# PRBonn/OverlapNet

Measured on NVIDIA H100. Metric: scan-pairs/sec (overlap+yaw) at 64x900, higher is better.
Workload: dtype f16

## Files before the change

overlapnet_b200/csrc/network_tc.cu:

```cuda
#include "common.cuh"
#include "hopper.cuh"

#include <cuda_fp16.h>
#include <stddef.h>
#include <stdlib.h>

namespace ovn {

using namespace hopper;

constexpr int WF = 360;
constexpr int CF = 128;
constexpr int S15 = 15;
constexpr int NB = 24;
constexpr int PAIR_ROWS = NB * NB;
constexpr int K4_PITCH = CF;

struct TcState {
  Buffer<__half> w1p;
  Buffer<__half> w2p;
  Buffer<__half> w3p;
  Buffer<float> b2eff;
  Buffer<__half> wres[kMaxLegLayers];
  Buffer<__half> actp[2];
// ... 23 lines not shown
};

void TcStateDelete::operator()(TcState* t) const { delete t; }

__host__ __device__ __forceinline__ int k4_pos(int r, int c) {
  const int k = c & 31;
  return (((c >> 5) ^ (r & 1)) << 5) + ((k & 7) >> 1) * 8 + (k >> 3) * 2 + (k & 1);
}

__device__ __forceinline__ bool h2_nonfinite(__half2 v) {
  const uint32_t b = *reinterpret_cast<const uint32_t*>(&v);
  return (b & 0x7c00u) == 0x7c00u || (b & 0x7c000000u) == 0x7c000000u;
}

__global__ void __launch_bounds__(256)
k_gather_rows_f16(const float* __restrict__ bank, const int32_t* __restrict__ idx, int n, const float* __restrict__ mu,
                  int row_shift, __half* __restrict__ out, int* __restrict__ err, int32_t* __restrict__ row_bad) {
  const int64_t per = (int64_t)WF * CF / 4;
  const int64_t i = (int64_t)blockIdx.x * blockDim.x + threadIdx.x;
  if (i >= (int64_t)n * per) return;
  const int p = (int)(i / per);
  const int64_t e = i % per;
  const int64_t row = idx ? idx[p] : p;
  const int r = (int)(e / (CF / 4)), c4 = (int)(e % (CF / 4));
  int64_t rs = r + row_shift;
  if (rs >= WF) rs -= WF;
  const float4 v = __ldg(reinterpret_cast<const float4*>(bank + (row * WF + rs) * CF) + c4);
  const float4 m = __ldg(reinterpret_cast<const float4*>(mu) + c4);
  __half2 a = __floats2half2_rn(v.x - m.x, v.y - m.y), b = __floats2half2_rn(v.z - m.z, v.w - m.w);
  if (h2_nonfinite(a) || h2_nonfinite(b)) {
    if (row_bad) row_bad[p] = 1;
    else atomicCAS(err, 0, kErrNonFiniteOperand);
  }
  __half* o = out + ((int64_t)p * WF + r) * K4_PITCH;
  *reinterpret_cast<uint32_t*>(o + k4_pos(r, 4 * c4)) = *reinterpret_cast<uint32_t*>(&a);
  *reinterpret_cast<uint32_t*>(o + k4_pos(r, 4 * c4 + 2)) = *reinterpret_cast<uint32_t*>(&b);
}

__global__ void __launch_bounds__(1024)
k_channel_mean(const float* __restrict__ bank, const int32_t* __restrict__ idx, int n, float* __restrict__ mu) {
  __shared__ float part[8][CF];
  const int c = threadIdx.x & (CF - 1), g = threadIdx.x >> 7;
  float acc = 0.f;
  for (int v = 0; v < n; ++v) {
    const float* vol = bank + (int64_t)(idx ? idx[v] : v) * WF * CF;
    for (int r = g; r < WF; r += 8) acc += __ldg(vol + (int64_t)r * CF + c);
  }
  part[g][c] = acc;
  __syncthreads();
  if (g == 0) {
    float t = 0.f;
    for (int k = 0; k < 8; ++k) t += part[k][c];
    mu[c] = __half2float(__float2half_rn(t / (float)((int64_t)n * WF)));
  }
}

constexpr int K4_STEPS = 60;

__host__ __device__ __forceinline__ size_t o1_row_offset(int64_t m, int di) {
  return ((size_t)((m >> 7) * S15 + di) * 128 + (size_t)(m & 127)) * 64;
}
__host__ __device__ __forceinline__ size_t o1_chunk_offset(int64_t m, int di, int c8) {
  return o1_row_offset(m, di) + (size_t)((c8 ^ (int)(m & 7)) * 8);
}

struct LegArgs {
  const __half* A; int64_t a_pitch;
  int runs_per_img, in_img_planes, in_run_planes;
  int kh, kw, c8in;
  const __half* Bp;
  const float* bias; int n_valid;
  int64_t M;
  __half* out_planes; int64_t out_pitch; int out_run_planes;
  float* out_f32;
  int n_split; float* part;
  int* err;
};

__device__ __forceinline__ bool leg_act_unstorable(float v) { return !(v < 65520.f) || v == -INFINITY; }

constexpr int C6_LROWS = 64, C6_RROWS = 128;
constexpr int C6_LT = 6, C6_RT = 3;
constexpr int C6_L_BYTES = 2 * 16 * C6_LROWS * 16;
constexpr int C6_R_BYTES = 2 * 16 * C6_RROWS * 16;
constexpr int C6_VOL_L_BYTES = C6_LT * C6_L_BYTES;
constexpr int C6_VOL_R_BYTES = C6_RT * C6_R_BYTES;

template <int TR, int NT>
__global__ void __launch_bounds__(256)
k_pack_corr(const float* __restrict__ bank, const int32_t* __restrict__ idx, int n, __half* __restrict__ out,
            int* __restrict__ err, int32_t* __restrict__ row_bad) {
  const int64_t i = (int64_t)blockIdx.x * blockDim.x + threadIdx.x;
  const int64_t per = 16 * NT * TR;
  if (i >= (int64_t)n * per) return;
  const int p = (int)(i / per);
  int r = (int)(i % per);
  const int vrow = r % (NT * TR); r /= NT * TR;
  const int pl = r;
  const int tile = vrow / TR, row = vrow % TR;
  float v[8];
  if (vrow < WF) {
    const int64_t src = (idx ? idx[p] : p);
    const float4 a = __ldg(reinterpret_cast<const float4*>(bank + (src * WF + vrow) * CF + pl * 8));
    const float4 b = __ldg(reinterpret_cast<const float4*>(bank + (src * WF + vrow) * CF + pl * 8 + 4));
    v[0] = a.x; v[1] = a.y; v[2] = a.z; v[3] = a.w; v[4] = b.x; v[5] = b.y; v[6] = b.z; v[7] = b.w;
  } else {
#pragma unroll
    for (int e = 0; e < 8; ++e) v[e] = 0.f;
  }
  __half hi[8], lo[8];
#pragma unroll
  for (int e = 0; e < 8; ++e) {
    hi[e] = __float2half_rn(v[e]);
    lo[e] = __float2half_rn(v[e] - __half2float(hi[e]));
  }
  bool bad = false;
#pragma unroll
  for (int e = 0; e < 8; e += 2) bad |= h2_nonfinite(__halves2half2(hi[e], hi[e + 1]));
  if (bad) {
    if (row_bad) row_bad[p] = 1;
    else atomicCAS(err, 0, kErrNonFiniteOperand);
  }
  __half* base = out + ((size_t)p * NT + tile) * (2 * 16 * TR * 8);
  *reinterpret_cast<uint4*>(base + ((size_t)pl * TR + row) * 8) = *reinterpret_cast<const uint4*>(hi);
  *reinterpret_cast<uint4*>(base + ((size_t)(16 + pl) * TR + row) * 8) = *reinterpret_cast<const uint4*>(lo);
}

constexpr int MMA_THREADS = 128;
constexpr int MMA_ROWS = 64;

__device__ __forceinline__ void mma16816(float (&d)[4], uint32_t a0, uint32_t a1, uint32_t a2, uint32_t a3,
                                         uint32_t b0, uint32_t b1) {
  asm volatile("mma.sync.aligned.m16n8k16.row.col.f32.f16.f16.f32 {%0,%1,%2,%3}, {%4,%5,%6,%7}, {%8,%9}, {%0,%1,%2,%3};"
               : "+f"(d[0]), "+f"(d[1]), "+f"(d[2]), "+f"(d[3])
               : "r"(a0), "r"(a1), "r"(a2), "r"(a3), "r"(b0), "r"(b1));
}

__device__ __forceinline__ uint32_t ld_h2(const __half* p) { return __ldg(reinterpret_cast<const unsigned int*>(p)); }

__device__ __forceinline__ uint32_t absdiff_h2(uint32_t a, uint32_t b) {
  const __half2 d = __hsub2(*reinterpret_cast<const __half2*>(&a), *reinterpret_cast<const __half2*>(&b));
  return *reinterpret_cast<const uint32_t*>(&d) & 0x7fff7fffu;
}

__device__ __forceinline__ uint32_t pack_h2(float a, float b) {
  const __half2 h = __floats2half2_rn(a, b);
  return *reinterpret_cast<const uint32_t*>(&h);
}

constexpr int K4_WG = 3;
constexpr int K4_THREADS = (K4_WG + 1) * 128;
constexpr uint32_t K4_REG_PRODUCER = 32, K4_REG_CONSUMER = 160;
constexpr int K4_GROUP = 5;
constexpr int K4_NGROUPS = K4_STEPS / K4_GROUP;
static_assert(S15 % K4_GROUP == 0, "a W1 group within one 32-channel chunk");
constexpr int K4_RING = 4;
constexpr int K4_BSLICE = 4096;
constexpr uint32_t K4_VOL_BYTES = WF * K4_PITCH * 2;
constexpr uint32_t K4_RWIN_BYTES = S15 * K4_PITCH * 2;
constexpr int K4_O1S_PITCH = NB * 64 + 8;

struct K4Smem {
  __half L[WF * K4_PITCH];
  __half Rw[2][S15 * K4_PITCH];
  __half B[K4_RING][K4_GROUP * K4_BSLICE / 2];
  __half O1s[S15 * K4_O1S_PITCH];
  MbarRing<K4_RING> w1;
  MbarRing<1> left;
  MbarRing<2> right;
  MbarRing<1> o1s;
};
static_assert(sizeof(K4Smem) <= 232448, "k_delta_conv1_wgmma shared memory");
static_assert(offsetof(K4Smem, B) % 16 == 0 && offsetof(K4Smem, Rw) % 16 == 0 && offsetof(K4Smem, O1s) % 16 == 0 &&
              K4_O1S_PITCH * 2 % 16 == 0, "bulk-copy alignment");

struct Share { int64_t begin, end; };
__device__ __forceinline__ Share work_share(int64_t n, uint32_t part, uint32_t parts) {
  return {n * part / parts, n * (part + 1) / parts};
}

__global__ void __launch_bounds__(K4_THREADS, 1)
k_delta_conv1_wgmma(const __half* __restrict__ L16, const int32_t* __restrict__ l_idx, const __half* __restrict__ R16,
                    int r_per_pair, const __half* __restrict__ W1p, const float* __restrict__ mu_o1,
                    __half* __restrict__ o1, int n_pairs, int* __restrict__ err) {
  extern __shared__ __align__(128) uint8_t smem_raw[];
  K4Smem& S = *reinterpret_cast<K4Smem*>(smem_raw);
  const int tid = threadIdx.x, warp = tid >> 5, lane = tid & 31;
  const Share share = work_share((int64_t)n_pairs * NB, blockIdx.x, gridDim.x);
  const int u_begin = (int)share.begin, u_end = (int)share.end;
  if (tid == 0) {
    S.w1.init(K4_WG * 4);
    S.left.init(K4_WG * 4);
    S.right.init(K4_WG * 4);
    S.o1s.init(1, K4_WG * 4);
    mbar_fence_init();
  }
  __syncthreads();

  if (warp >= K4_WG * 4) {
    setmaxnreg_dec<K4_REG_PRODUCER>();
    if (warp == K4_WG * 4 && lane == 0) {
      uint32_t pi = 0, gi = 0, ui = 0;
      for (int u = u_begin; u < u_end; ++u, ++ui) {
        const int p = u / NB, jb = u - p * NB;
        if (u == u_begin || jb == 0) {
          PIPE_WAIT(S.left.acquire(pi, K4_VOL_BYTES), kErrDeltaLeftProducer);
          bulk_g2s(S.L, L16 + (size_t)(l_idx ? l_idx[p] : p) * WF * K4_PITCH, K4_VOL_BYTES, S.left.bar(pi));
          ++pi;
        }
        PIPE_WAIT(S.right.acquire(ui, K4_RWIN_BYTES), kErrDeltaRightProducer);
        bulk_g2s(S.Rw[S.right.slot(ui)], R16 + (r_per_pair ? (size_t)p * WF * K4_PITCH : 0) + (size_t)jb * S15 * K4_PITCH,
                 K4_RWIN_BYTES, S.right.bar(ui));
        for (int grp = 0; grp < K4_NGROUPS; ++grp, ++gi) {
          PIPE_WAIT(S.w1.acquire(gi, K4_GROUP * K4_BSLICE), kErrDeltaW1Producer);
          bulk_g2s(S.B[S.w1.slot(gi)], W1p + (size_t)grp * K4_GROUP * (K4_BSLICE / 2), K4_GROUP * K4_BSLICE, S.w1.bar(gi));
        }
      }
    } else if (warp == K4_WG * 4 + 1 && lane == 0) {
      uint32_t ui = 0;
      for (int u = u_begin; u < u_end; ++u, ++ui) {
        const int p = u / NB, jb = u - p * NB;
        const int64_t m0 = (int64_t)p * PAIR_ROWS + jb * NB;
        const int n0 = min(NB, 128 - (int)(m0 & 127));
        if (!S.o1s.wait(ui)) { atomicExch(err, kErrDeltaO1Producer); break; }
#pragma unroll 1
        for (int di = 0; di < S15; ++di) {
          const __half* src = S.O1s + di * K4_O1S_PITCH;
          bulk_s2g(o1 + o1_row_offset(m0, di), src, n0 * 128);
          if (n0 < NB) bulk_s2g(o1 + o1_row_offset(m0 + n0, di), src + n0 * 64, (NB - n0) * 128);
        }
        bulk_commit();
        bulk_wait_read<0>();
        S.o1s.release_thread(ui);
      }
      bulk_wait<0>();
    }
  } else {
    setmaxnreg_inc<K4_REG_CONSUMER>();
    const int wg = warp >> 2, wi = warp & 3, g = lane >> 2, t = lane & 3;
    int rows[2][2];
#pragma unroll
    for (int tt = 0; tt < 2; ++tt) {
      const int r = (wg + 3 * tt) * 64 + wi * 16 + g;
      rows[tt][0] = r;
      rows[tt][1] = r + 8;
    }
    const uint32_t b_base = smem_u32(S.B[0]);
    uint32_t pi = 0, gi = 0, ui = 0;
    for (int u = u_begin; u < u_end; ++u, ++ui) {
      const int p = u / NB, jb = u - p * NB;
      if (u == u_begin || jb == 0) { PIPE_WAIT(S.left.wait(pi), kErrDeltaLeftConsumer); ++pi; }
      const uint32_t wb = S.right.slot(ui);
      PIPE_WAIT(S.right.wait(ui), kErrDeltaRightConsumer);
      float acc[2][32];
#pragma unroll
      for (int j = 0; j < 8; ++j) {
        const float m0 = __half2float(__float2half_rn(-__ldg(mu_o1 + j * 8 + 2 * t)));
        const float m1 = __half2float(__float2half_rn(-__ldg(mu_o1 + j * 8 + 2 * t + 1)));
#pragma unroll
        for (int tt = 0; tt < 2; ++tt) {
          acc[tt][4 * j + 0] = m0; acc[tt][4 * j + 1] = m1;
          acc[tt][4 * j + 2] = m0; acc[tt][4 * j + 3] = m1;
        }
      }
      uint32_t Lr[2][2][4];
#pragma unroll 1
      for (int grp = 0; grp < K4_NGROUPS; ++grp, ++gi) {
        const int cc = grp / 3, dj0 = (grp - 3 * cc) * K4_GROUP;
        if (dj0 == 0) {
#pragma unroll
          for (int tt = 0; tt < 2; ++tt)
#pragma unroll
            for (int h = 0; h < 2; ++h) {
              const int r = rows[tt][h] < WF ? rows[tt][h] : WF - 1;
              const uint4 v = *reinterpret_cast<const uint4*>(S.L + r * K4_PITCH + ((cc ^ (r & 1)) << 5) + 8 * t);
              Lr[tt][h][0] = v.x; Lr[tt][h][1] = v.y; Lr[tt][h][2] = v.z; Lr[tt][h][3] = v.w;
            }
        }
        const uint32_t s = S.w1.slot(gi);
        const uint64_t bdesc = desc_kmajor(b_base + s * (K4_GROUP * K4_BSLICE), 1024, 128, kNoSwizzle);
        const int par = (jb + dj0) & 1;
        const __half* rw = S.Rw[wb] + dj0 * K4_PITCH + 8 * t;
        const __half* rp[2] = {rw + ((cc ^ par) << 5), rw + ((cc ^ par ^ 1) << 5)};
        uint4 rv = *reinterpret_cast<const uint4*>(rp[0]);
        PIPE_WAIT(S.w1.wait(gi), kErrDeltaW1Consumer);
        uint32_t A[2][2][4];
#pragma unroll
        for (int sl = 0; sl < K4_GROUP; ++sl)
#pragma unroll
          for (int kk = 0; kk < 2; ++kk) {
            const uint32_t r0 = kk ? rv.z : rv.x, r1 = kk ? rv.w : rv.y;
#pragma unroll
            for (int tt = 0; tt < 2; ++tt) {
              A[tt][kk][0] = absdiff_h2(Lr[tt][0][2 * kk], r0);
              A[tt][kk][1] = absdiff_h2(Lr[tt][1][2 * kk], r0);
              A[tt][kk][2] = absdiff_h2(Lr[tt][0][2 * kk + 1], r1);
              A[tt][kk][3] = absdiff_h2(Lr[tt][1][2 * kk + 1], r1);
            }
            wgmma_fence();
#pragma unroll
            for (int tt = 0; tt < 2; ++tt)
              wgmma_m64n64k16_rs(acc[tt], A[tt][kk], bdesc + ((sl * K4_BSLICE + kk * 2048) >> 4));
            wgmma_commit();
            if (kk == 1 && sl + 1 < K4_GROUP) rv = *reinterpret_cast<const uint4*>(rp[(sl + 1) & 1] + (sl + 1) * K4_PITCH);
            wgmma_wait<1>();
          }
        wgmma_wait<0>();
        S.w1.release(gi);
      }
      S.right.release(ui);
      if (jb == NB - 1 || u == u_end - 1) S.left.release(pi - 1);
      if (!S.o1s.wait_free(ui)) { atomicExch(err, kErrDeltaO1Consumer); goto done; }
#pragma unroll
      for (int tt = 0; tt < 2; ++tt)
#pragma unroll
        for (int h = 0; h < 2; ++h) {
          const int i = rows[tt][h];
          if (i >= WF) continue;
          const int ibk = i / S15, di = i - ibk * S15;
          __half* st = S.O1s + di * K4_O1S_PITCH + ibk * 64 + 2 * t;
#pragma unroll
          for (int j = 0; j < 8; ++j)
            *reinterpret_cast<uint32_t*>(st + ((j ^ (ibk & 7)) << 3)) =
                pack_h2(acc[tt][4 * j + 2 * h], acc[tt][4 * j + 2 * h + 1]);
        }
      fence_proxy_async_smem();
      S.o1s.publish(ui);
    }
  }
done:
  return;
}

constexpr int TC_WG = 2;
constexpr int TC_THREADS = TC_WG * 128 + 32;
constexpr int TC_ROWS = TC_WG * 128;
constexpr uint32_t C2_TILE = 128 * 64 * 2;
constexpr int C2_RING = 3;

struct C2Smem {
  __half A[C2_RING][TC_WG][C2_TILE / 2];
  __half B[C2_RING][2][C2_TILE / 2];
  MbarRing<C2_RING> ring;
};
constexpr size_t C2_SMEM = sizeof(C2Smem) + 1024;
static_assert(C2_SMEM <= 232448, "k_conv2_wgmma shared memory");
static_assert(offsetof(C2Smem, B) % 1024 == 0 && C2_TILE % 1024 == 0, "SWIZZLE_128B tiles on 1024-byte boundaries");

__global__ void __launch_bounds__(TC_THREADS, 1)
k_conv2_wgmma(const __half* __restrict__ o1, const __half* __restrict__ W2s, const float* __restrict__ bias2,
              const float* __restrict__ mu_x3, __half* __restrict__ x3, int64_t out_pitch, int64_t M, int fault,
              int* __restrict__ err) {
  if (fault) {
    if (threadIdx.x == 0 && blockIdx.x == 0) atomicExch(err, kErrInjectedFault);
    return;
  }
  extern __shared__ __align__(128) uint8_t smem_raw[];
  C2Smem& S = *reinterpret_cast<C2Smem*>(smem_raw + ((1024 - (smem_u32(smem_raw) & 1023)) & 1023));
  const int tid = threadIdx.x, warp = tid >> 5, lane = tid & 31;
  const Share tiles = work_share((M + TC_ROWS - 1) / TC_ROWS, blockIdx.x, gridDim.x);
  if (tid == 0) {
    S.ring.init(TC_WG * 4);
    mbar_fence_init();
  }
  __syncthreads();

  if (warp == TC_WG * 4) {
    if (lane == 0) {
      uint32_t gi = 0;
      for (int64_t tile = tiles.begin; tile < tiles.end; ++tile)
        for (int di = 0; di < S15; ++di, ++gi) {
          const uint32_t s = S.ring.slot(gi);
          PIPE_WAIT(S.ring.acquire(gi, 4 * C2_TILE), kErrConv2Producer);
          for (int h = 0; h < TC_WG; ++h)
            bulk_g2s(S.A[s][h], o1 + ((size_t)(tile * TC_WG + h) * S15 + di) * (C2_TILE / 2), C2_TILE, S.ring.bar(gi));
          bulk_g2s(S.B[s], W2s + (size_t)di * C2_TILE, 2 * C2_TILE, S.ring.bar(gi));
        }
    }
  } else {
    const int wg = warp >> 2, wi = warp & 3, g = lane >> 2, t = lane & 3;
    uint32_t gi = 0;
    bool failed = false;
    for (int64_t tile = tiles.begin; tile < tiles.end; ++tile) {
      float acc[2][64];
#pragma unroll
      for (int sub = 0; sub < 2; ++sub)
#pragma unroll
        for (int e = 0; e < 64; ++e) acc[sub][e] = 0.f;
#pragma unroll 1
      for (int di = 0; di < S15; ++di, ++gi) {
        const uint32_t s = S.ring.slot(gi);
        INFLIGHT_WAIT(S.ring.wait(gi), kErrConv2Consumer);
        const uint32_t a_base = smem_u32(S.A[s][wg]), b_base = smem_u32(S.B[s][0]);
        wgmma_fence();
#pragma unroll
        for (int kk = 0; kk < 4; ++kk)
#pragma unroll
          for (int part = 0; part < 2; ++part) {
            const uint64_t bd = desc_kmajor(b_base + part * C2_TILE + kk * 32, 16, 1024, kSwizzle128B);
#pragma unroll
            for (int sub = 0; sub < 2; ++sub)
              wgmma_m64n128k16_ss(acc[sub], desc_kmajor(a_base + sub * (C2_TILE / 2) + kk * 32, 16, 1024, kSwizzle128B), bd);
          }
        wgmma_commit();
        wgmma_wait<1>();
        if (di > 0) S.ring.release(gi - 1);
      }
      wgmma_wait<0>();
      if (failed) goto done;
      S.ring.release(gi - 1);
#pragma unroll
      for (int sub = 0; sub < 2; ++sub)
#pragma unroll
        for (int h = 0; h < 2; ++h) {
          const int64_t m = tile * TC_ROWS + wg * 128 + sub * 64 + wi * 16 + g + 8 * h;
          if (m >= M) continue;
#pragma unroll
          for (int j = 0; j < 16; ++j) {
            const int n = j * 8 + 2 * t;
            const float a = fmaxf(acc[sub][4 * j + 2 * h] + __ldg(bias2 + n), 0.f) - __ldg(mu_x3 + n);
            const float b = fmaxf(acc[sub][4 * j + 2 * h + 1] + __ldg(bias2 + n + 1), 0.f) - __ldg(mu_x3 + n + 1);
            *reinterpret_cast<uint32_t*>(x3 + ((size_t)j * out_pitch + m) * 8 + 2 * t) = pack_h2(a, b);
          }
        }
    }
  }
done:
  return;
}

constexpr int C3_AROWS = TC_ROWS + 2 * NB + 2;
constexpr uint32_t C3_PLANE = C3_AROWS * 16;
constexpr uint32_t C3_SLAB = 4 * 128 * 16;
constexpr int C3_GROUP = 2;
constexpr int C3_NSTAGES = 36 / C3_GROUP;
constexpr int C3_RING = 4;

struct C3Smem {
  __half A[2][16 * C3_PLANE / 2];
  __half B[C3_RING][C3_GROUP * C3_SLAB / 2];
  MbarRing<C3_RING> w3;
  MbarRing<2> x3;
};
static_assert(sizeof(C3Smem) <= 232448, "k_conv3_wgmma shared memory");
static_assert(offsetof(C3Smem, B) % 16 == 0 && C3_PLANE % 16 == 0, "bulk-copy alignment");

__global__ void __launch_bounds__(TC_THREADS, 1)
k_conv3_wgmma(const __half* __restrict__ X3, int64_t a_pitch, const __half* __restrict__ W3p, const float* __restrict__ bias,
              int64_t M, const float* __restrict__ wd, float* __restrict__ partial, int* __restrict__ err) {
  extern __shared__ __align__(128) uint8_t smem_raw[];
  C3Smem& S = *reinterpret_cast<C3Smem*>(smem_raw);
  const int tid = threadIdx.x, warp = tid >> 5, lane = tid & 31;
  const Share tiles = work_share(2 * ((M + TC_ROWS - 1) / TC_ROWS), blockIdx.x, gridDim.x);
  if (tid == 0) {
    S.w3.init(TC_WG * 4);
    S.x3.init(TC_WG * 4);
    mbar_fence_init();
  }
  __syncthreads();

  if (warp == TC_WG * 4) {
    if (lane == 0) {
      const uint32_t nt = (uint32_t)(tiles.end - tiles.begin);
      uint32_t ai = 0, gi = 0;
      for (uint32_t ti = 0; ti < nt; ++ti) {
        const int nh = (int)((tiles.begin + ti) & 1);
        for (int st = 0; st < C3_NSTAGES; ++st, ++gi) {
          while (ai < nt && ai <= ti + 1) {
            if (ai > ti) {
              if (!S.x3.try_acquire(ai, 16 * C3_PLANE)) break;
            } else {
              PIPE_WAIT(S.x3.acquire(ai, 16 * C3_PLANE), kErrConv3X3Producer);
            }
            const int64_t r0 = ((tiles.begin + ai) >> 1) * TC_ROWS;
            for (int pl = 0; pl < 16; ++pl)
              bulk_g2s(S.A[S.x3.slot(ai)] + pl * (C3_PLANE / 2), X3 + ((size_t)pl * a_pitch + r0) * 8, C3_PLANE, S.x3.bar(ai));
            ++ai;
// ... 767 lines not shown
  return OVN_OK;
}

int tc_bank_prepare(ovn_handle* h, const float* d_bank, int64_t capacity, int64_t first, int64_t count, cudaStream_t s) {
  TcState* t = h->tc.get();
  if (!t) OVN_SET_ERR(h, OVN_ERR_WEIGHTS, "tensor-core weights not packed");
  const size_t l16_bytes = (size_t)capacity * WF * K4_PITCH * sizeof(__half);
  if (t->pb_key != d_bank || l16_bytes > t->pb_l16.bytes()) {
    int rc = OVN_OK;
    if (t->pb_key != nullptr || t->pb_l16) rc = tc_bank_release(h, nullptr);
    if (rc == OVN_OK) rc = t->pb_l16.ensure(h, l16_bytes);
    if (rc == OVN_OK) rc = t->pb_lc.ensure(h, (size_t)capacity * C6_VOL_L_BYTES);
    if (rc == OVN_OK) rc = t->pb_bad.ensure(h, (size_t)capacity * sizeof(int32_t));
    if (rc != OVN_OK) return rc;
    OVN_CUDA(h, cudaMemsetAsync(t->pb_l16, 0, l16_bytes, s));
    t->pb_key = d_bank;
    t->pb_rows = 0;
    if (first != 0) OVN_SET_ERR(h, OVN_ERR_INVALID_ARG, "ovn_bank_prepare: a new bank must be prepared from row 0");
  }
  if (first > t->pb_rows) OVN_SET_ERR(h, OVN_ERR_INVALID_ARG, "ovn_bank_prepare: rows [%lld, %lld) were never prepared",
                                      (long long)t->pb_rows, (long long)first);
  const int64_t per = (int64_t)WF * CF / 4, perL = 16 * C6_LT * C6_LROWS;
  const float* src = d_bank + (size_t)first * WF * CF;
  if (!t->mu_set) {
    int rc = calibrate_all(h, src, nullptr, false, s);
    if (rc != OVN_OK) return rc;
  }
  OVN_CUDA(h, cudaMemsetAsync(t->pb_bad + first, 0, (size_t)count * sizeof(int32_t), s));
  k_gather_rows_f16<<<(unsigned)((count * per + 255) / 256), 256, 0, s>>>(src, nullptr, (int)count, t->mu, 0,
                                                                         t->pb_l16 + (size_t)first * WF * K4_PITCH, h->d_err,
                                                                         t->pb_bad + first);
  OVN_LAUNCH_CHECK(h);
  k_pack_corr<C6_LROWS, C6_LT><<<(unsigned)((count * perL + 255) / 256), 256, 0, s>>>(src, nullptr, (int)count,
                                                                      t->pb_lc + (size_t)first * (C6_VOL_L_BYTES / 2), h->d_err,
                                                                      t->pb_bad + first);
  OVN_LAUNCH_CHECK(h);
  if (first + count > t->pb_rows) t->pb_rows = first + count;
  return OVN_OK;
}

static int calibrate_all(ovn_handle* h, const float* d_vols, const int32_t* d_idx, bool keep_mu, cudaStream_t s) {
  TcState* t = h->tc.get();
  const int base = kMaxLegLayers;
  const int64_t per = (int64_t)WF * CF / 4;
  if (!keep_mu) {
    k_channel_mean<<<1, 1024, 0, s>>>(d_vols, d_idx, 1, t->mu);
    OVN_LAUNCH_CHECK(h);
  }
  OVN_CUDA(h, cudaMemsetAsync(t->mu_o1, 0, 64 * sizeof(float), s));
  OVN_CUDA(h, cudaMemsetAsync(t->mu_x3, 0, 128 * sizeof(float), s));
  k_gather_rows_f16<<<(unsigned)((per + 255) / 256), 256, 0, s>>>(d_vols, d_idx, 1, t->mu, 0, t->l16, h->d_err, nullptr);
  OVN_LAUNCH_CHECK(h);
  k_gather_rows_f16<<<(unsigned)((per + 255) / 256), 256, 0, s>>>(d_vols, d_idx, 1, t->mu, WF / 2, t->r16, h->d_err, nullptr);
  OVN_LAUNCH_CHECK(h);
  t->last_n = 0;
  const int64_t Mc = PAIR_ROWS;
  const int g4c = NB < h->sm_count ? NB : h->sm_count;
  const int64_t tiles_c = (Mc + TC_ROWS - 1) / TC_ROWS;
  k_delta_conv1_wgmma<<<g4c, K4_THREADS, sizeof(K4Smem), s>>>(t->l16, nullptr, t->r16, 0, t->w1p, t->mu_o1, t->o1, 1, h->d_err);
  OVN_LAUNCH_CHECK(h);
  k_o1_channel_mean<<<1, 1024, 0, s>>>(t->o1, Mc, t->mu_o1);
  OVN_LAUNCH_CHECK(h);
  k_fold_bias2<<<1, 128, 0, s>>>(t->b2base, t->mu_o1, h->d_w[base + 1], t->b2eff);
  OVN_LAUNCH_CHECK(h);
  k_delta_conv1_wgmma<<<g4c, K4_THREADS, sizeof(K4Smem), s>>>(t->l16, nullptr, t->r16, 0, t->w1p, t->mu_o1, t->o1, 1, h->d_err);
  OVN_LAUNCH_CHECK(h);
  k_conv2_wgmma<<<(unsigned)tiles_c, TC_THREADS, C2_SMEM, s>>>(t->o1, t->w2p, t->b2eff, t->mu_x3, t->x3, t->rows_pad, Mc, 0,
                                                              h->d_err);
  OVN_LAUNCH_CHECK(h);
  k_x3_channel_mean<<<1, 1024, 0, s>>>(t->x3, t->rows_pad, Mc, t->mu_x3);
  OVN_LAUNCH_CHECK(h);
  k_fold_bias3<<<1, 256, 0, s>>>(h->d_b[base + 2], t->mu_x3, h->d_w[base + 2], t->b3eff);
  OVN_LAUNCH_CHECK(h);
  t->mu_set = true;
  t->act_set = true;
  return OVN_OK;
}

int tc_calibrate(ovn_handle* h, const float* d_volume, cudaStream_t s) {
  TcState* t = h->tc.get();
  if (!t) OVN_SET_ERR(h, OVN_ERR_WEIGHTS, "tensor-core weights not packed");
  if (t->pb_key != nullptr)
    OVN_SET_ERR(h, OVN_ERR_INVALID_ARG, "ovn_calibrate: release the resident bank first (its operand copies were built "
                "with the previous centre)");
  return calibrate_all(h, d_volume, nullptr, false, s);
}

int tc_set_center(ovn_handle* h, const float* h_mu) {
  TcState* t = h->tc.get();
  if (!t) OVN_SET_ERR(h, OVN_ERR_WEIGHTS, "tensor-core weights not packed");
  if (t->pb_key != nullptr)
    OVN_SET_ERR(h, OVN_ERR_INVALID_ARG, "ovn_set_feature_center: release the resident bank first (its operand copies "
                "were built with the previous centre)");
  OVN_CUDA(h, cudaDeviceSynchronize());
  t->act_set = false;
  OVN_CUDA(h, cudaMemset(t->mu_o1, 0, 64 * sizeof(float)));
  OVN_CUDA(h, cudaMemset(t->mu_x3, 0, 128 * sizeof(float)));
  if (!h_mu) {
    t->mu_set = false;
    OVN_CUDA(h, cudaMemset(t->mu, 0, CF * sizeof(float)));
    return OVN_OK;
  }
  float m[CF];
  for (int c = 0; c < CF; ++c) m[c] = __half2float(__float2half(h_mu[c]));
  OVN_CUDA(h, cudaMemcpy(t->mu, m, sizeof(m), cudaMemcpyHostToDevice));
  t->mu_set = true;
  return OVN_OK;
}

int tc_get_center(ovn_handle* h, float* h_mu, int32_t* is_set) {
  TcState* t = h->tc.get();
  if (!t) OVN_SET_ERR(h, OVN_ERR_WEIGHTS, "tensor-core weights not packed");
  OVN_CUDA(h, cudaDeviceSynchronize());
  OVN_CUDA(h, cudaMemcpy(h_mu, t->mu, CF * sizeof(float), cudaMemcpyDeviceToHost));
  *is_set = t->mu_set ? 1 : 0;
  return OVN_OK;
}

int heads_forward_tc(ovn_handle* h, const float* d_bank, const float* d_query, const int32_t* d_left,
                     const int32_t* d_right, int n, float* d_overlap, int32_t* d_yaw, float* d_corr,
                     cudaStream_t s) {
  TcState* t = h->tc.get();
  if (!t) OVN_SET_ERR(h, OVN_ERR_WEIGHTS, "tensor-core weights not packed");
  const int maxp = h->cfg.max_batch_pairs;
  const int base = kMaxLegLayers;
  const int64_t per = (int64_t)WF * CF / 4;
  t->last_n = 0;
  if ((!t->mu_set || !t->act_set) && n > 0) {
    int rc = d_query ? calibrate_all(h, d_query, nullptr, t->mu_set, s) : calibrate_all(h, d_bank, d_right, t->mu_set, s);
    if (rc != OVN_OK) return rc;
  }
  const bool resident = (t->pb_key == d_bank) && t->pb_rows > 0;
  const __half* l16 = resident ? t->pb_l16 : t->l16;
  const __half* lc = resident ? t->pb_lc : t->lc;
  int32_t* lidx = nullptr;
  if (resident) {
    lidx = h->d_idx_san + 2 * (size_t)maxp;
    int rc = sanitize_indices(h, d_left, n, t->pb_rows, kErrRowNotPrepared, lidx, s, t->pb_bad);
    if (rc != OVN_OK) return rc;
  } else {
    k_gather_rows_f16<<<(unsigned)((n * per + 255) / 256), 256, 0, s>>>(d_bank, d_left, n, t->mu, 0, t->l16, h->d_err, nullptr);
    OVN_LAUNCH_CHECK(h);
  }
  if (d_query)
    k_gather_rows_f16<<<(unsigned)((per + 255) / 256), 256, 0, s>>>(d_query, nullptr, 1, t->mu, 0, t->r16, h->d_err, nullptr);
  else
    k_gather_rows_f16<<<(unsigned)((n * per + 255) / 256), 256, 0, s>>>(d_bank, d_right, n, t->mu, 0, t->r16, h->d_err, nullptr);
  OVN_LAUNCH_CHECK(h);
  const int64_t M = (int64_t)n * PAIR_ROWS;
  const int64_t tiles = (M + TC_ROWS - 1) / TC_ROWS;
  const int grid2 = tiles < h->sm_count ? (int)tiles : h->sm_count;
  const int grid3 = 2 * tiles < h->sm_count ? (int)(2 * tiles) : h->sm_count;
  prof_mark(h, PROF_DELTA, s);
  const int64_t units = (int64_t)n * NB;
  const int grid4 = units < h->sm_count ? (int)units : h->sm_count;
  k_delta_conv1_wgmma<<<grid4, K4_THREADS, sizeof(K4Smem), s>>>(l16, lidx, t->r16, d_query ? 0 : 1, t->w1p, t->mu_o1, t->o1,
                                                               n, h->d_err);
  prof_mark(h, PROF_DELTA, s);
  OVN_LAUNCH_CHECK(h);
  const bool inject_fault = getenv("OVN_DEBUG_FAULT") != nullptr;
  prof_mark(h, PROF_CONV2, s);
  k_conv2_wgmma<<<grid2, TC_THREADS, C2_SMEM, s>>>(t->o1, t->w2p, t->b2eff, t->mu_x3, t->x3, t->rows_pad, M,
                                                   inject_fault ? 1 : 0, h->d_err);
  prof_mark(h, PROF_CONV2, s);
  OVN_LAUNCH_CHECK(h);
  prof_mark(h, PROF_CONV3, s);
  k_conv3_wgmma<<<grid3, TC_THREADS, sizeof(C3Smem), s>>>(t->x3, t->rows_pad, t->w3p, t->b3eff, M, h->d_w[base + 3],
                                                          t->partial, h->d_err);
  prof_mark(h, PROF_CONV3, s);
  OVN_LAUNCH_CHECK(h);
  k_dense_finalize<<<n, 256, 0, s>>>(t->partial, h->d_b[base + 3], PAIR_ROWS, d_overlap, h->d_err);
  OVN_LAUNCH_CHECK(h);
  const int64_t perL = 16 * C6_LT * C6_LROWS, perR = 16 * C6_RT * C6_RROWS;
  if (!resident) {
    k_pack_corr<C6_LROWS, C6_LT><<<(unsigned)((n * perL + 255) / 256), 256, 0, s>>>(d_bank, d_left, n, t->lc, h->d_err, nullptr);
    OVN_LAUNCH_CHECK(h);
  }
  if (d_query)
    k_pack_corr<C6_RROWS, C6_RT><<<(unsigned)((perR + 255) / 256), 256, 0, s>>>(d_query, nullptr, 1, t->rc, h->d_err, nullptr);
  else
    k_pack_corr<C6_RROWS, C6_RT><<<(unsigned)((n * perR + 255) / 256), 256, 0, s>>>(d_bank, d_right, n, t->rc, h->d_err, nullptr);
  OVN_LAUNCH_CHECK(h);
  prof_mark(h, PROF_CORR, s);
  const int nc = (int64_t)n * C6_LT < h->sm_count / C6_RT ? n * C6_LT : h->sm_count / C6_RT;
  k_corr_wgmma<<<nc * C6_RT, C6_THREADS, sizeof(C6Smem), s>>>(lc, lidx, t->rc, d_query ? 0 : 1, n, t->corr_part, h->d_err);
  prof_mark(h, PROF_CORR, s);
  OVN_LAUNCH_CHECK(h);
  k_corr_finalize<<<n, 384, 0, s>>>(t->corr_part, d_corr, d_yaw, h->d_err);
  OVN_LAUNCH_CHECK(h);
  t->last_n = n;
  static const bool debug_sync = getenv("OVN_DEBUG_SYNC") != nullptr;
  if (debug_sync) return check_device_error(h, s);
  return OVN_OK;
}

__global__ void __launch_bounds__(256)
k_copy_heads_stage(int stage, const __half* __restrict__ o1, const __half* __restrict__ x3, int64_t x3_pitch,
                   const float* __restrict__ partial, int64_t first, int64_t total, float* __restrict__ out) {
  const int64_t e = (int64_t)blockIdx.x * blockDim.x + threadIdx.x;
  if (e >= total) return;
  out += e;
  if (stage == OVN_STAGE_O1) {
    const int o = (int)(e % 64), jb = (int)(e / 64 % NB), i = (int)(e / (64 * NB) % WF);
    const int64_t p = first + e / (64 * NB * WF);
    const int64_t m = p * PAIR_ROWS + jb * NB + i / S15;
    *out = __half2float(o1[o1_chunk_offset(m, i % S15, o >> 3) + (o & 7)]);
  } else if (stage == OVN_STAGE_X3) {
    const int c = (int)(e % 128), jb = (int)(e / 128 % NB), ib = (int)(e / (128 * NB) % NB);
    const int64_t m = (first + e / (128 * PAIR_ROWS)) * PAIR_ROWS + jb * NB + ib;
    *out = __half2float(x3[((size_t)(c >> 3) * x3_pitch + m) * 8 + (c & 7)]);
  } else {
    const int half = (int)(e % 2), jb = (int)(e / 2 % NB), ib = (int)(e / (2 * NB) % NB);
    const int64_t m = (first + e / (2 * PAIR_ROWS)) * PAIR_ROWS + jb * NB + ib;
    *out = partial[m * 2 + half];
  }
}

int64_t tc_heads_stage_pairs(const ovn_handle* h) {
  const TcState* t = h->tc.get();
  return t ? t->last_n : 0;
}

int tc_copy_heads_stage(ovn_handle* h, int stage, int64_t first, int64_t count, float* d_out, cudaStream_t s) {
  TcState* t = h->tc.get();
  if (!t || t->last_n == 0)
    OVN_SET_ERR(h, OVN_ERR_INVALID_ARG, "ovn_copy_heads_stage: no stored stages (no complete heads call since the "
                "weights were packed or the centres calibrated)");
  if (!d_out) OVN_SET_ERR(h, OVN_ERR_INVALID_ARG, "ovn_copy_heads_stage: NULL pointer");
  if (stage != OVN_STAGE_CENTRES && (first < 0 || count < 1 || first + count > t->last_n))
    OVN_SET_ERR(h, OVN_ERR_INVALID_ARG, "ovn_copy_heads_stage: pairs [%lld, %lld) outside the %lld stored",
                (long long)first, (long long)(first + count), (long long)t->last_n);
  if (stage == OVN_STAGE_CENTRES) {
    const Buffer<float>* parts[4] = {&t->mu_o1, &t->mu_x3, &t->b2eff, &t->b3eff};
    const size_t len[4] = {64, 128, 128, 256};
    for (int k = 0; k < 4; ++k) {
      OVN_CUDA(h, cudaMemcpyAsync(d_out, *parts[k], len[k] * sizeof(float), cudaMemcpyDeviceToDevice, s));
      d_out += len[k];
    }
    return OVN_OK;
  }
  const int64_t per = stage == OVN_STAGE_O1 ? (int64_t)WF * NB * 64 : stage == OVN_STAGE_X3 ? PAIR_ROWS * 128 : PAIR_ROWS * 2;
  const int64_t total = count * per;
  k_copy_heads_stage<<<(unsigned)((total + 255) / 256), 256, 0, s>>>(stage, t->o1, t->x3, t->rows_pad, t->partial, first,
                                                                       total, d_out);
  OVN_LAUNCH_CHECK(h);
  return OVN_OK;
}

__global__ void __launch_bounds__(256)
k_copy_leg_stage(const __half* __restrict__ planes, int w_out, int cout, int64_t total, float* __restrict__ hi,
                 float* __restrict__ lo) {
  const int64_t e = (int64_t)blockIdx.x * blockDim.x + threadIdx.x;
  if (e >= total) return;
  const int c = (int)(e % cout), x = (int)(e / cout % w_out);
  const int64_t row = e / cout / w_out;
  const int c8n = cout / 8;
  const __half* p = planes + ((size_t)(row * 2 * c8n + (c >> 3)) * w_out + x) * 8 + (c & 7);
  hi[e] = __half2float(p[0]);
  lo[e] = __half2float(p[(size_t)c8n * w_out * 8]);
}

int tc_leg_stage(ovn_handle* h, const float* d_input, int n, int layer, float* d_hi, float* d_lo, cudaStream_t s) {
  const int rc = leg_forward_tc(h, d_input, n, nullptr, s, layer);
  if (rc != OVN_OK) return rc;
  const ConvSpec& L = h->leg[layer];
  const int64_t total = (int64_t)n * L.h_out * L.w_out * L.cout;
  k_copy_leg_stage<<<(unsigned)((total + 255) / 256), 256, 0, s>>>(h->tc->actp[layer & 1], L.w_out, L.cout, total, d_hi, d_lo);
  OVN_LAUNCH_CHECK(h);
  return OVN_OK;
}

}
```

Baseline: 211,200.

## Pack left rows across pairs into full 384-row blocks in delta conv1 kernel

When a single query is compared against many bank scans, the conv1 delta kernel now processes blocks of 384 consecutive left rows that can span pair boundaries, instead of one 360-row pair per block. This fills the 2x3 wgmma M tiles that previously sat partly idle, and the right window and W1 stream are shared across more useful rows. The O1 store-out becomes per-lane parallel over the 15 shifts, and the smem store addresses are precomputed once per block. The W1 ring shrinks from 4 to 3 stages to fit the larger staging buffers. Indexing becomes more complex, with multi-segment bulk copies and extra boundary handling.

```diff
diff --git a/overlapnet_b200/csrc/network_tc.cu b/overlapnet_b200/csrc/network_tc.cu
--- a/overlapnet_b200/csrc/network_tc.cu
+++ b/overlapnet_b200/csrc/network_tc.cu
@@ -199,16 +199,29 @@
 constexpr int K4_THREADS = (K4_WG + 1) * 128;
 constexpr uint32_t K4_REG_PRODUCER = 32, K4_REG_CONSUMER = 160;
 constexpr int K4_GROUP = 5;
+constexpr int K4_CHUNK_GROUPS = S15 / K4_GROUP;
 constexpr int K4_NGROUPS = K4_STEPS / K4_GROUP;
 static_assert(S15 % K4_GROUP == 0, "a W1 group within one 32-channel chunk");
-constexpr int K4_RING = 4;
+constexpr int K4_RING = 3;
 constexpr int K4_BSLICE = 4096;
-constexpr uint32_t K4_VOL_BYTES = WF * K4_PITCH * 2;
+constexpr int K4_BLOCK_ROWS = 2 * K4_WG * 64;
 constexpr uint32_t K4_RWIN_BYTES = S15 * K4_PITCH * 2;
-constexpr int K4_O1S_PITCH = NB * 64 + 8;
+static_assert(WF % NB == 0 && K4_BLOCK_ROWS % NB == 0, "blocks start on a multiple of 24 rows");
+constexpr int K4_O1S_Q = (K4_BLOCK_ROWS + S15 - 2) / S15 + 1;
+constexpr int K4_O1S_PITCH = K4_O1S_Q * 64 + 8;
+
+struct K4Block { int g0, rows; };
+__host__ __device__ __forceinline__ int k4_blocks(int n_pairs, int r_per_pair) {
+  return r_per_pair ? n_pairs : (n_pairs * WF + K4_BLOCK_ROWS - 1) / K4_BLOCK_ROWS;
+}
+__device__ __forceinline__ K4Block k4_block(int b, int r_per_pair, int n_pairs) {
+  if (r_per_pair) return {b * WF, WF};
+  const int g0 = b * K4_BLOCK_ROWS;
+  return {g0, min(K4_BLOCK_ROWS, n_pairs * WF - g0)};
+}
 
 struct K4Smem {
-  __half L[WF * K4_PITCH];
+  __half L[K4_BLOCK_ROWS * K4_PITCH];
   __half Rw[2][S15 * K4_PITCH];
   __half B[K4_RING][K4_GROUP * K4_BSLICE / 2];
   __half O1s[S15 * K4_O1S_PITCH];
@@ -233,7 +246,7 @@
   extern __shared__ __align__(128) uint8_t smem_raw[];
   K4Smem& S = *reinterpret_cast<K4Smem*>(smem_raw);
   const int tid = threadIdx.x, warp = tid >> 5, lane = tid & 31;
-  const Share share = work_share((int64_t)n_pairs * NB, blockIdx.x, gridDim.x);
+  const Share share = work_share((int64_t)k4_blocks(n_pairs, r_per_pair) * NB, blockIdx.x, gridDim.x);
   const int u_begin = (int)share.begin, u_end = (int)share.end;
   if (tid == 0) {
     S.w1.init(K4_WG * 4);
@@ -249,38 +262,54 @@
     if (warp == K4_WG * 4 && lane == 0) {
       uint32_t pi = 0, gi = 0, ui = 0;
       for (int u = u_begin; u < u_end; ++u, ++ui) {
-        const int p = u / NB, jb = u - p * NB;
+        const int b = u / NB, jb = u - b * NB;
         if (u == u_begin || jb == 0) {
-          PIPE_WAIT(S.left.acquire(pi, K4_VOL_BYTES), kErrDeltaLeftProducer);
-          bulk_g2s(S.L, L16 + (size_t)(l_idx ? l_idx[p] : p) * WF * K4_PITCH, K4_VOL_BYTES, S.left.bar(pi));
+          const K4Block blk = k4_block(b, r_per_pair, n_pairs);
+          const int p = blk.g0 / WF, i0 = blk.g0 - p * WF, n1 = min(blk.rows, WF - i0);
+          PIPE_WAIT(S.left.acquire(pi, blk.rows * K4_PITCH * 2), kErrDeltaLeftProducer);
+          bulk_g2s(S.L, L16 + ((size_t)(l_idx ? l_idx[p] : p) * WF + i0) * K4_PITCH, n1 * K4_PITCH * 2, S.left.bar(pi));
+          if (n1 < blk.rows)
+            bulk_g2s(S.L + n1 * K4_PITCH, L16 + (size_t)(l_idx ? l_idx[p + 1] : p + 1) * WF * K4_PITCH,
+                     (blk.rows - n1) * K4_PITCH * 2, S.left.bar(pi));
           ++pi;
         }
         PIPE_WAIT(S.right.acquire(ui, K4_RWIN_BYTES), kErrDeltaRightProducer);
-        bulk_g2s(S.Rw[S.right.slot(ui)], R16 + (r_per_pair ? (size_t)p * WF * K4_PITCH : 0) + (size_t)jb * S15 * K4_PITCH,
+        bulk_g2s(S.Rw[S.right.slot(ui)], R16 + (r_per_pair ? (size_t)b * WF * K4_PITCH : 0) + (size_t)jb * S15 * K4_PITCH,
                  K4_RWIN_BYTES, S.right.bar(ui));
         for (int grp = 0; grp < K4_NGROUPS; ++grp, ++gi) {
           PIPE_WAIT(S.w1.acquire(gi, K4_GROUP * K4_BSLICE), kErrDeltaW1Producer);
           bulk_g2s(S.B[S.w1.slot(gi)], W1p + (size_t)grp * K4_GROUP * (K4_BSLICE / 2), K4_GROUP * K4_BSLICE, S.w1.bar(gi));
         }
       }
-    } else if (warp == K4_WG * 4 + 1 && lane == 0) {
+    } else if (warp == K4_WG * 4 + 1) {
+      const int di = lane;
       uint32_t ui = 0;
       for (int u = u_begin; u < u_end; ++u, ++ui) {
-        const int p = u / NB, jb = u - p * NB;
-        const int64_t m0 = (int64_t)p * PAIR_ROWS + jb * NB;
-        const int n0 = min(NB, 128 - (int)(m0 & 127));
-        if (!S.o1s.wait(ui)) { atomicExch(err, kErrDeltaO1Producer); break; }
+        const int b = u / NB, jb = u - b * NB;
+        const K4Block blk = k4_block(b, r_per_pair, n_pairs);
+        if (!__all_sync(0xffffffffu, S.o1s.wait(ui))) {
+          if (lane == 0) atomicExch(err, kErrDeltaO1Producer);
+          break;
+        }
+        if (di < S15) {
+          const int q0 = blk.g0 / S15, qb = (blk.g0 + blk.rows - 1 - di) / S15;
 #pragma unroll 1
-        for (int di = 0; di < S15; ++di) {
-          const __half* src = S.O1s + di * K4_O1S_PITCH;
-          bulk_s2g(o1 + o1_row_offset(m0, di), src, n0 * 128);
-          if (n0 < NB) bulk_s2g(o1 + o1_row_offset(m0 + n0, di), src + n0 * 64, (NB - n0) * 128);
-        }
-        bulk_commit();
-        bulk_wait_read<0>();
-        S.o1s.release_thread(ui);
-      }
-      bulk_wait<0>();
+          for (int q = (blk.g0 + S15 - 1 - di) / S15; q <= qb;) {
+            const int p = q / NB, ib = q - p * NB, len = min(qb - q + 1, NB - ib);
+            const int64_t m = (int64_t)p * PAIR_ROWS + jb * NB + ib;
+            const int n0 = min(len, 128 - (int)(m & 127));
+            const __half* src = S.O1s + di * K4_O1S_PITCH + (q - q0) * 64;
+            bulk_s2g(o1 + o1_row_offset(m, di), src, n0 * 128);
+            if (n0 < len) bulk_s2g(o1 + o1_row_offset(m + n0, di), src + n0 * 64, (len - n0) * 128);
+            q += len;
+          }
+          bulk_commit();
+          bulk_wait_read<0>();
+        }
+        __syncwarp();
+        if (lane == 0) S.o1s.release_thread(ui);
+      }
+      if (di < S15) bulk_wait<0>();
     }
   } else {
     setmaxnreg_inc<K4_REG_CONSUMER>();
@@ -294,9 +323,23 @@
     }
     const uint32_t b_base = smem_u32(S.B[0]);
     uint32_t pi = 0, gi = 0, ui = 0;
+    uint32_t sto[2][2][8];
     for (int u = u_begin; u < u_end; ++u, ++ui) {
-      const int p = u / NB, jb = u - p * NB;
-      if (u == u_begin || jb == 0) { PIPE_WAIT(S.left.wait(pi), kErrDeltaLeftConsumer); ++pi; }
+      const int b = u / NB, jb = u - b * NB;
+      const K4Block blk = k4_block(b, r_per_pair, n_pairs);
+      if (u == u_begin || jb == 0) {
+        PIPE_WAIT(S.left.wait(pi), kErrDeltaLeftConsumer);
+        ++pi;
+#pragma unroll
+        for (int tt = 0; tt < 2; ++tt)
+#pragma unroll
+          for (int h = 0; h < 2; ++h) {
+            const int g = blk.g0 + rows[tt][h], q = g / S15, di = g - q * S15, ib = q % NB;
+            const uint32_t st = (uint32_t)offsetof(K4Smem, O1s) + 2 * (di * K4_O1S_PITCH + (q - blk.g0 / S15) * 64 + 2 * t);
+#pragma unroll
+            for (int j = 0; j < 8; ++j) sto[tt][h][j] = st + ((j ^ (ib & 7)) << 4);
+          }
+      }
       const uint32_t wb = S.right.slot(ui);
       PIPE_WAIT(S.right.wait(ui), kErrDeltaRightConsumer);
       float acc[2][32];
@@ -313,13 +356,13 @@
       uint32_t Lr[2][2][4];
 #pragma unroll 1
       for (int grp = 0; grp < K4_NGROUPS; ++grp, ++gi) {
-        const int cc = grp / 3, dj0 = (grp - 3 * cc) * K4_GROUP;
+        const int cc = grp / K4_CHUNK_GROUPS, dj0 = (grp - K4_CHUNK_GROUPS * cc) * K4_GROUP;
         if (dj0 == 0) {
 #pragma unroll
           for (int tt = 0; tt < 2; ++tt)
 #pragma unroll
             for (int h = 0; h < 2; ++h) {
-              const int r = rows[tt][h] < WF ? rows[tt][h] : WF - 1;
+              const int r = rows[tt][h] < blk.rows ? rows[tt][h] : blk.rows - 1;
               const uint4 v = *reinterpret_cast<const uint4*>(S.L + r * K4_PITCH + ((cc ^ (r & 1)) << 5) + 8 * t);
               Lr[tt][h][0] = v.x; Lr[tt][h][1] = v.y; Lr[tt][h][2] = v.z; Lr[tt][h][3] = v.w;
             }
@@ -362,14 +405,10 @@
       for (int tt = 0; tt < 2; ++tt)
 #pragma unroll
         for (int h = 0; h < 2; ++h) {
-          const int i = rows[tt][h];
-          if (i >= WF) continue;
-          const int ibk = i / S15, di = i - ibk * S15;
-          __half* st = S.O1s + di * K4_O1S_PITCH + ibk * 64 + 2 * t;
+          if (rows[tt][h] >= blk.rows) continue;
 #pragma unroll
           for (int j = 0; j < 8; ++j)
-            *reinterpret_cast<uint32_t*>(st + ((j ^ (ibk & 7)) << 3)) =
-                pack_h2(acc[tt][4 * j + 2 * h], acc[tt][4 * j + 2 * h + 1]);
+            *reinterpret_cast<uint32_t*>(smem_raw + sto[tt][h][j]) = pack_h2(acc[tt][4 * j + 2 * h], acc[tt][4 * j + 2 * h + 1]);
         }
       fence_proxy_async_smem();
       S.o1s.publish(ui);
@@ -1443,7 +1482,7 @@
   const int grid2 = tiles < h->sm_count ? (int)tiles : h->sm_count;
   const int grid3 = 2 * tiles < h->sm_count ? (int)(2 * tiles) : h->sm_count;
   prof_mark(h, PROF_DELTA, s);
-  const int64_t units = (int64_t)n * NB;
+  const int64_t units = (int64_t)k4_blocks(n, d_query ? 0 : 1) * NB;
   const int grid4 = units < h->sm_count ? (int)units : h->sm_count;
   k_delta_conv1_wgmma<<<grid4, K4_THREADS, sizeof(K4Smem), s>>>(l16, lidx, t->r16, d_query ? 0 : 1, t->w1p, t->mu_o1, t->o1,
                                                                n, h->d_err);
```

Result: faster. 219,800 (median of 6 runs) (+4.1%).
